# google/neural-light-transport

Hardware: NVIDIA B200
Metric: UV texels/sec fwd+bwd (higher is better)
Workload: dtype f32

## Files before the change

neural-light-transport_b200/csrc/nlt_tc.cu:

```cuda
#include <cuda.h>
#include "nlt_common.cuh"

namespace nlt {

constexpr int TC_MAX_STAGES = 8;
constexpr int TC_BM = 128;
constexpr int TC_EPI_PAD = 36;
constexpr int TC_EPI_BYTES = 4 * 32 * TC_EPI_PAD * 4;
constexpr int TC_THREADS = 320;
constexpr int TCF_THREADS = 448;
constexpr uint32_t TC_SPIN_LIMIT = 1u << 28;
unsigned long long g_tc_launches = 0;

int g_opt_tc_rawhi = -1;

struct TcParams {
  int N, Hl, Wl;
  int TW, TH;
  int tiles_x, tiles_y;
  int n_tiles_n;
  int total_tiles;
  int ntap_y, ntap_x;
  int nseg;
  int seg_chunks[NLT_MAX_SEG];
// ... 604 lines not shown
    const int lq = lane % QPR, lr = lane / QPR;

    struct Coord { int n, ty0, tx0, nt; };
    auto tile_coord = [&](int tile) {
      Coord c;
      const int mt = (int)fdiv((uint32_t)tile, p.div_ntn);
      c.nt = tile - mt * p.n_tiles_n;
      c.n = (int)fdiv((uint32_t)mt, p.div_tpi);
      const int r = mt - c.n * tiles_per_img;
      const int rq = (int)fdiv((uint32_t)r, p.div_tx);
      c.ty0 = rq * p.TH; c.tx0 = (r - rq * p.tiles_x) * p.TW;
      return c;
    };
    auto out_off = [&](const Coord& c, int row, int nb) -> size_t {
      const int rty = (int)fdiv((uint32_t)row, p.div_tw);
      const int ty = c.ty0 + rty, tx = c.tx0 + row - rty * p.TW;
      int cb = nb, oy, ox;
      if (p.d2s) {
        const int tap = (int)fdiv((uint32_t)nb, p.div_ct);
        cb = nb - tap * p.cout_true;
        const int dy = (int)fdiv((uint32_t)tap, p.div_s);
        oy = ty * p.d2s_s + dy; ox = tx * p.d2s_s + (tap - dy * p.d2s_s);
      } else {
        oy = p.o0y + p.osy * ty; ox = p.o0x + p.osx * tx;
      }
      return (((size_t)c.n * p.Hout + oy) * p.Wout + ox) * p.cout_true + cb;
    };
    float4 rm_old[NPASS], rm_y[NPASS];
    auto prefetch = [&](const Coord& c, int ch) {
#pragma unroll
      for (int i = 0; i < NPASS; ++i) {
        const size_t ob = out_off(c, quarter * 32 + i * RPI + lr, c.nt * BN + ch * 32 + lq * 4);
        rm_old[i] = (p.beta != 0.f) ? *reinterpret_cast<const float4*>(p.out + ob) : make_float4(0.f, 0.f, 0.f, 0.f);
        rm_y[i] = (p.mask_y != nullptr) ? ld4(p.mask_y + ob) : make_float4(1.f, 1.f, 1.f, 1.f);
      }
    };
    int it = 0;
    for (int tile = blockIdx.x; tile < p.total_tiles; tile += gridDim.x, ++it) {
      const int buf = it & 1;
      const uint32_t acc_phase = (uint32_t)(it >> 1) & 1;
      const Coord tc = tile_coord(tile);
      const uint32_t taddr = tmem_base + ((uint32_t)(quarter * 32) << 16) + (uint32_t)(buf * BN);
#pragma unroll 1
      for (int ch = 0; ch < NCH; ++ch) {
        if (rmw) prefetch(tc, ch);
        if (ch == 0) {
          mbar_wait(bar_accf(buf), acc_phase);
          tc_fence_after();
        }
        const int col0 = tc.nt * BN + ch * 32;
#pragma unroll
        for (int h = 0; h < CW / 16; ++h) {
          uint32_t v[16];
          tc_ld16(taddr + ch * 32 + h * 16, v);
#pragma unroll
          for (int q4 = 0; q4 < 4; ++q4) {
            int cb = col0 + h * 16 + q4 * 4;
            if (p.d2s) cb -= (int)fdiv((uint32_t)cb, p.div_ct) * p.cout_true;
            float o[4];
#pragma unroll
            for (int e = 0; e < 4; ++e) {
              float x = __uint_as_float(v[q4 * 4 + e]);
              if (p.bias != nullptr) x += __ldg(p.bias + cb + e);
              o[e] = act_fwd(x, p.act);
            }
            *reinterpret_cast<float4*>(stg + lane * TC_EPI_PAD + h * 16 + q4 * 4) = make_float4(o[0], o[1], o[2], o[3]);
          }
        }
        __syncwarp();
#pragma unroll
        for (int i = 0; i < NPASS; ++i) {
          const int row = i * RPI + lr;
          float4 o = *reinterpret_cast<const float4*>(stg + row * TC_EPI_PAD + lq * 4);
          if (rmw) {
            o.x += p.beta * rm_old[i].x; o.y += p.beta * rm_old[i].y; o.z += p.beta * rm_old[i].z; o.w += p.beta * rm_old[i].w;
            if (p.mask_y != nullptr) {
              o.x *= act_bwd_from_y(rm_y[i].x, p.mask_act); o.y *= act_bwd_from_y(rm_y[i].y, p.mask_act);
              o.z *= act_bwd_from_y(rm_y[i].z, p.mask_act); o.w *= act_bwd_from_y(rm_y[i].w, p.mask_act);
            }
          }
          const size_t ob = out_off(tc, quarter * 32 + row, col0 + lq * 4);
          *reinterpret_cast<float4*>(p.out + ob) = o;
        }
        __syncwarp();
      }
      tc_fence_before();
      mbar_arrive(bar_acce(buf));
    }
  }

  tc_fence_before();
  __syncthreads();
  if (warp == 1) {
    tc_fence_after();
    asm volatile("tcgen05.dealloc.cta_group::1.sync.aligned.b32 %0, %1;" ::"r"(tmem_base), "r"(TMEM_COLS) : "memory");
  }
}

typedef CUresult (*EncodeTiledFn)(CUtensorMap*, CUtensorMapDataType, cuuint32_t, void*, const cuuint64_t*,
                                  const cuuint64_t*, const cuuint32_t*, const cuuint32_t*, CUtensorMapInterleave,
                                  CUtensorMapSwizzle, CUtensorMapL2promotion, CUtensorMapFloatOOBfill);

static EncodeTiledFn get_encode() {
  static EncodeTiledFn fn = nullptr;
  static bool tried = false;
  if (!tried) {
    tried = true;
    void* sym = nullptr;
    cudaDriverEntryPointQueryResult qres;
    if (cudaGetDriverEntryPoint("cuTensorMapEncodeTiled", &sym, cudaEnableDefault, &qres) == cudaSuccess &&
        qres == cudaDriverEntryPointSuccess)
      fn = (EncodeTiledFn)sym;
  }
  return fn;
}

struct TcPlan {
  bool ok;
  bool ts;
  int bn;
  int kbw;
  TcParams p;
  int chunks_per_tap;
  int cout_pad;
  size_t pack_floats;
  size_t smem_bytes;
};

static int pick_bn(int cout) {
  if (cout % 128 == 0) return 128;
  if (cout % 64 == 0) return 64;
  if (cout % 32 == 0) return 32;
  if (cout % 16 == 0) return 16;
  return 0;
}

int g_opt_tcs = -1;
static int g_tcs_kmin = -1;
static bool tcs_enabled() {
  if (g_opt_tcs < 0) { const char* e = getenv("NLT_TCS"); g_opt_tcs = e ? (atoi(e) != 0) : NLT_TCS_DEFAULT; }
  if (g_tcs_kmin < 0) { const char* e = getenv("NLT_TCS_KMIN"); g_tcs_kmin = e ? atoi(e) : 64; }
  return g_opt_tcs == 1;
}

static TcPlan tc_plan(const GConvK& k) {
  TcPlan pl;
  memset(&pl, 0, sizeof(pl));
  pl.ok = false;
  const bool ts = tcs_enabled();
  pl.ts = ts;
  if (k.cout_true % 4 != 0) return pl;
  pl.bn = pick_bn(k.Cout);
  if (pl.bn == 0) return pl;
  int ctot = 0;
  pl.kbw = 32;
  for (int s = 0; s < k.nseg; ++s) {
    const Seg& sg = k.seg[s];
    if (sg.C % 16 != 0 || sg.sub != nullptr || sg.bcast || !aligned16(sg.ptr)) return pl;
    if (sg.C % 32 != 0) pl.kbw = 16;
    ctot += sg.C;
  }
  const int TC_KB = pl.kbw;
  if (!aligned16(k.w)) {  }
  if (ts) {
    if (k.ay.nu * k.ax.nu * ctot < g_tcs_kmin) return pl;
  } else {
    if (k.ay.nu * k.ax.nu * ctot < 64) return pl;
    if (pl.kbw == 16 && k.ay.nu * k.ax.nu * ctot < 128) return pl;
  }
  if (k.ay.nu < 1 || k.ax.nu < 1) return pl;
  TcParams& p = pl.p;
  p.N = k.N; p.Hl = k.ay.nt; p.Wl = k.ax.nt;
  if (p.Wl >= TC_BM) {
    if (p.Wl % TC_BM) return pl;
    p.TW = TC_BM; p.TH = 1;
  } else {
    if (TC_BM % p.Wl) return pl;
    p.TW = p.Wl; p.TH = TC_BM / p.Wl;
    if (p.Hl % p.TH) return pl;
  }
  p.tiles_x = p.Wl / p.TW; p.tiles_y = p.Hl / p.TH;
  const bool stride1 = (k.ay.it == 1 && k.ax.it == 1);
  const bool patch = (!k.d2s && k.ay.it > 1 && k.ay.it == k.ax.it && k.ay.iu == 1 && k.ax.iu == 1 && k.ay.i0 == 0 &&
                      k.ax.i0 == 0 && k.ay.nu == k.ay.it && k.ax.nu == k.ax.it && k.Hin == k.ay.nt * k.ay.it &&
                      k.Win == k.ax.nt * k.ax.it);
  if (!stride1 && !patch) return pl;
  p.mode_patch = patch ? 1 : 0;
  p.ux_step = k.ax.iu; p.x_off = k.ax.i0; p.uy_step = k.ay.iu; p.y_off = k.ay.i0;
  p.Hs = patch ? k.Hin / k.ay.it : 0;
  if (patch && (k.ay.it > 256 || p.TW > 256)) return pl;
  p.ntap_y = k.ay.nu; p.ntap_x = k.ax.nu;
  p.nseg = k.nseg;
  pl.chunks_per_tap = 0;
  for (int s = 0; s < k.nseg; ++s) { p.seg_chunks[s] = k.seg[s].C / TC_KB; pl.chunks_per_tap += p.seg_chunks[s]; }
  p.kb_total = p.ntap_y * p.ntap_x * pl.chunks_per_tap;
  p.Hout = k.Hout; p.Wout = k.Wout; p.cout_true = k.cout_true; p.Cout = k.Cout;
  p.o0y = k.ay.o0; p.osy = k.ay.os; p.o0x = k.ax.o0; p.osx = k.ax.os;
  p.d2s = k.d2s; p.d2s_s = k.d2s_s;
  static int split_waves = -1;
  if (split_waves < 0) { const char* e = getenv("NLT_TC_SPLIT_WAVES"); split_waves = (e && e[0] == '1') ? 1 : 0; }
  while (pl.bn > 32) {
    const long long tiles = (long long)p.N * p.tiles_x * p.tiles_y * (k.Cout / pl.bn);
    if (split_waves ? tiles >= 148 : 2 * tiles > 148) break;
    pl.bn /= 2;
  }
  p.n_tiles_n = k.Cout / pl.bn;
  p.div_ntn = make_fastdiv((uint32_t)p.n_tiles_n); p.div_tpi = make_fastdiv((uint32_t)(p.tiles_x * p.tiles_y));
  p.div_tx = make_fastdiv((uint32_t)p.tiles_x); p.div_tw = make_fastdiv((uint32_t)p.TW);
  p.div_ct = make_fastdiv((uint32_t)p.cout_true); p.div_s = make_fastdiv((uint32_t)(p.d2s ? p.d2s_s : 1));
  const long long tt = (long long)p.N * p.tiles_x * p.tiles_y * p.n_tiles_n;
  if (tt > (1ll << 30)) return pl;
  p.total_tiles = (int)tt;
  pl.cout_pad = k.Cout;
  pl.pack_floats = (size_t)p.kb_total * pl.cout_pad * TC_KB;
  {
    const size_t stage_bytes = (ts ? 1 : 2) * (size_t)TC_BM * TC_KB * 4 + 2 * (size_t)pl.bn * TC_KB * 4;
    int st = (int)((227 * 1024 - TC_EPI_BYTES - 2048) / stage_bytes);
    if (st > TC_MAX_STAGES) st = TC_MAX_STAGES;
    if (st < 2) return pl;
    p.stages = st;
    pl.smem_bytes = (size_t)st * stage_bytes + TC_EPI_BYTES + 1024;
  }
  if (get_encode() == nullptr) return pl;
  {
    static int ablate = -1;
    if (ablate < 0) {
      const char* e = getenv("NLT_TC_ABLATE");
      ablate = e ? atoi(e) : 0;
      if (ablate & 32) { const int one = 1; cudaMemcpyToSymbol(g_tc_poll, &one, sizeof(int)); }
    }
    p.ablate = ablate;
    if (g_opt_tc_rawhi < 0) { const char* e = getenv("NLT_TC_RAWHI"); g_opt_tc_rawhi = (e && e[0] == '0') ? 0 : 1; }
    p.rawhi = g_opt_tc_rawhi;
  }
  pl.ok = true;
  return pl;
}

static int encode_maps(const GConvK& k, const TcPlan& pl, const float* bhi, const float* blo, TcMaps* maps) {
  EncodeTiledFn enc = get_encode();
  const TcParams& p = pl.p;
  const int TC_KB = pl.kbw;
  const CUtensorMapSwizzle swz = pl.kbw == 32 ? CU_TENSOR_MAP_SWIZZLE_128B : CU_TENSOR_MAP_SWIZZLE_64B;
  for (int s = 0; s < k.nseg; ++s) {
    const Seg& sg = k.seg[s];
    const cuuint64_t C = sg.C, W = k.Win, H = k.Hin, N = k.N;
    CUresult r;
    if (p.mode_patch) {
      const cuuint64_t st = k.ay.it;
      cuuint64_t dims[5] = {C, st, W / st, st, N * (H / st)};
      cuuint64_t strides[4] = {C * 4, st * C * 4, W * C * 4, st * W * C * 4};
      cuuint32_t box[5] = {(cuuint32_t)TC_KB, 1, (cuuint32_t)p.TW, 1, (cuuint32_t)p.TH};
      cuuint32_t es[5] = {1, 1, 1, 1, 1};
      r = enc(&maps->a[s], CU_TENSOR_MAP_DATA_TYPE_FLOAT32, 5, (void*)sg.ptr, dims, strides, box, es,
              CU_TENSOR_MAP_INTERLEAVE_NONE, swz, CU_TENSOR_MAP_L2_PROMOTION_L2_128B,
              CU_TENSOR_MAP_FLOAT_OOB_FILL_NONE);
    } else {
      cuuint64_t dims[4] = {C, W, H, N};
      cuuint64_t strides[3] = {C * 4, W * C * 4, H * W * C * 4};
      cuuint32_t box[4] = {(cuuint32_t)TC_KB, (cuuint32_t)p.TW, (cuuint32_t)p.TH, 1};
      cuuint32_t es[4] = {1, 1, 1, 1};
      r = enc(&maps->a[s], CU_TENSOR_MAP_DATA_TYPE_FLOAT32, 4, (void*)sg.ptr, dims, strides, box, es,
              CU_TENSOR_MAP_INTERLEAVE_NONE, swz, CU_TENSOR_MAP_L2_PROMOTION_L2_128B,
              CU_TENSOR_MAP_FLOAT_OOB_FILL_NONE);
    }
    if (r != CUDA_SUCCESS) return set_err(NLT_ERR_CUDA, "cuTensorMapEncodeTiled(A seg %d) failed: %d", s, (int)r);
  }
  const float* planes[2] = {bhi, blo};
  CUtensorMap* bm[2] = {&maps->bhi, &maps->blo};
  for (int i = 0; i < 2; ++i) {
    cuuint64_t dims[3] = {(cuuint64_t)TC_KB, (cuuint64_t)pl.cout_pad, (cuuint64_t)p.kb_total};
    cuuint64_t strides[2] = {(cuuint64_t)TC_KB * 4, (cuuint64_t)TC_KB * 4 * pl.cout_pad};
    cuuint32_t box[3] = {(cuuint32_t)TC_KB, (cuuint32_t)pl.bn, 1};
    cuuint32_t es[3] = {1, 1, 1};
    CUresult r = enc(bm[i], CU_TENSOR_MAP_DATA_TYPE_FLOAT32, 3, (void*)planes[i], dims, strides, box, es,
                     CU_TENSOR_MAP_INTERLEAVE_NONE, swz, CU_TENSOR_MAP_L2_PROMOTION_L2_256B,
                     CU_TENSOR_MAP_FLOAT_OOB_FILL_NONE);
    if (r != CUDA_SUCCESS) return set_err(NLT_ERR_CUDA, "cuTensorMapEncodeTiled(B) failed: %d", (int)r);
  }
  return NLT_OK;
}

constexpr int WG_PT = 32;
constexpr int WG_MAX_PIECES = 36;
constexpr int WG_PLANE_A = TC_BM * 128;

struct WgPiece {
  int16_t is_g, seg, uy, ux;
  int16_t c0, w;
  int16_t row, pad;
  int32_t raw_off;
};

struct WgParams {
  int N, Hl, Wl, TW, TH, tiles_x, tiles_y, total_ptiles;
  int mode_patch, ux_step, x_off, uy_step, y_off, Hs;
  int g_patch, g_px, g_py, g_Hs;
  int g_ct, g_s;
  int ntap_x, nseg, ctot, Kd;
  int seg_C[NLT_MAX_SEG], seg_coff[NLT_MAX_SEG];
  int n_mtiles, n_ntiles;
  FastDiv div_tpi, div_tx;
  int raw_stages, raw_stage_bytes;
  int Cout, ld, KD_pad, bias_row;
  float* ws;
};

struct WgMaps {
  CUtensorMap a[NLT_MAX_SEG][4];
  CUtensorMap g;
};

__device__ __forceinline__ int wg_wclass(int w) { return w == 32 ? 3 : w == 16 ? 2 : w == 8 ? 1 : 0; }

__device__ __forceinline__ int wg_raw_chunk(int w, int p, int cq) {
  return w == 32 ? (cq ^ (p & 7)) : w == 16 ? (cq ^ ((p >> 1) & 3)) : w == 8 ? (cq ^ ((p >> 2) & 1)) : cq;
}

template <int BN>
__global__ void __launch_bounds__(TC_THREADS, 1)
tc_wgrad_kernel(const __grid_constant__ WgMaps maps, const WgParams p) {
  constexpr int PLANE_G = BN * 128;
  constexpr int PLANES_BYTES = 2 * WG_PLANE_A + 2 * PLANE_G;
  constexpr uint32_t TMEM_COLS = BN <= 32 ? 32 : BN <= 64 ? 64 : 128;
  constexpr uint32_t IDESC = (1u << 4) | (2u << 7) | (2u << 10) | ((uint32_t)(BN >> 3) << 17) | ((uint32_t)(TC_BM >> 4) << 24);
  constexpr int GQ = BN / 4;
  constexpr int GI = (GQ + 3) / 4;

  extern __shared__ uint8_t smem_raw[];
  uint8_t* smem = smem_raw + ((1024u - (smem_u32(smem_raw) & 1023u)) & 1023u);
  __shared__ __align__(8) uint64_t bars[2 * TC_MAX_STAGES + 5];
  __shared__ uint32_t tmem_base_smem;
  __shared__ WgPiece pieces[WG_MAX_PIECES];
  __shared__ uint16_t items[64];
  __shared__ int n_pieces_s, n_items_s, raw_bytes_s;
  __shared__ float bias_part[64];

  const int S = p.raw_stages;
  const int warp = threadIdx.x >> 5, lane = threadIdx.x & 31;
  const uint32_t bar0 = smem_u32(bars);
  auto bar_rfull = [&](int s) { return bar0 + 8u * s; };
  auto bar_rempty = [&](int s) { return bar0 + 8u * (TC_MAX_STAGES + s); };
  auto bar_tready = [&](int b) { return bar0 + 8u * (2 * TC_MAX_STAGES + b); };
  auto bar_tempty = [&](int b) { return bar0 + 8u * (2 * TC_MAX_STAGES + 2 + b); };
  const uint32_t bar_accf = bar0 + 8u * (2 * TC_MAX_STAGES + 4);
  uint8_t* planes = smem;
  uint8_t* raw = smem + 2 * PLANES_BYTES;
  const uint32_t planes_u32 = smem_u32(planes), raw_u32 = smem_u32(raw);

  const int mtile = blockIdx.y, ntile = blockIdx.z;
  const int k_lo = mtile * TC_BM, k_hi = min(p.Kd, k_lo + TC_BM);

  if (threadIdx.x == 0) {
    int np = 0, off = 0, k = k_lo;
    while (k < k_hi) {
      const int tap = k / p.ctot, c = k - tap * p.ctot;
      int s = 0;
      while (s < p.nseg - 1 && c >= p.seg_coff[s] + p.seg_C[s]) ++s;
      const int cin = c - p.seg_coff[s];
      int w = p.seg_C[s] - cin;
      if (w > 32) w = 32;
      if (w > k_hi - k) w = k_hi - k;
      w = w >= 32 ? 32 : w >= 16 ? 16 : w >= 8 ? 8 : 4;
      WgPiece& pc = pieces[np++];
      pc.is_g = 0; pc.seg = (int16_t)s; pc.uy = (int16_t)(tap / p.ntap_x); pc.ux = (int16_t)(tap % p.ntap_x);
      pc.c0 = (int16_t)cin; pc.w = (int16_t)w; pc.row = (int16_t)(k - k_lo); pc.pad = 0; pc.raw_off = off;
      off += (WG_PT * w * 4 + 1023) & ~1023;
      k += w;
    }
    const int gw = p.g_patch == 2 ? min(min(BN, 32), p.g_ct) : (BN < 32 ? BN : 32);
    for (int c = 0; c < BN; c += gw) {
      WgPiece& pc = pieces[np++];
      pc.is_g = 1; pc.seg = 0; pc.uy = 0; pc.ux = 0; pc.c0 = (int16_t)(ntile * BN + c); pc.w = (int16_t)gw;
      if (p.g_patch == 2) {
        const int ncol = ntile * BN + c, tap = ncol / p.g_ct;
        pc.c0 = (int16_t)(ncol - tap * p.g_ct);
        pc.uy = (int16_t)(tap / p.g_s); pc.ux = (int16_t)(tap % p.g_s);
      }
      pc.row = (int16_t)c; pc.pad = 0; pc.raw_off = off;
      off += (WG_PT * gw * 4 + 1023) & ~1023;
    }
    n_pieces_s = np;
    int bytes = 0, ni = 0;
    for (int i = 0; i < np; ++i) {
      bytes += WG_PT * pieces[i].w * 4;
      for (int cq = 0; cq < pieces[i].w / 4; ++cq) items[ni++] = (uint16_t)((i << 8) | cq);
    }
    n_items_s = ni;
    raw_bytes_s = bytes;
    for (int s = 0; s < S; ++s) { mbar_init(bar_rfull(s), 1); mbar_init(bar_rempty(s), 8); }
    for (int b = 0; b < 2; ++b) { mbar_init(bar_tready(b), 8); mbar_init(bar_tempty(b), 1); }
    mbar_init(bar_accf, 1);
    asm volatile("fence.mbarrier_init.release.cluster;" ::: "memory");
  }
  for (int i = threadIdx.x; i < 2 * PLANES_BYTES / 16; i += TC_THREADS)
    reinterpret_cast<float4*>(planes)[i] = make_float4(0.f, 0.f, 0.f, 0.f);
  if (warp == 1) {
    asm volatile("tcgen05.alloc.cta_group::1.sync.aligned.shared::cta.b32 [%0], %1;" ::"r"(smem_u32(&tmem_base_smem)),
                 "r"(TMEM_COLS) : "memory");
    asm volatile("tcgen05.relinquish_alloc_permit.cta_group::1.sync.aligned;" ::: "memory");
  }
  asm volatile("fence.proxy.async.shared::cta;" ::: "memory");
  tc_fence_before();
  __syncthreads();
  tc_fence_after();
  const uint32_t tmem_base = tmem_base_smem;
  const int n_pieces = n_pieces_s;
  const int tiles_per_img = p.tiles_x * p.tiles_y;
  int my_tiles = 0;
  for (int t = blockIdx.x; t < p.total_ptiles; t += gridDim.x) ++my_tiles;

  if (warp == 0) {
    if (lane == 0) {
      int stage = 0;
      uint32_t phase = 0;
      for (int t = blockIdx.x; t < p.total_ptiles; t += gridDim.x) {
        const int n = (int)fdiv((uint32_t)t, p.div_tpi);
        const int r = t - n * tiles_per_img;
        const int rq = (int)fdiv((uint32_t)r, p.div_tx);
        const int ty0 = rq * p.TH, tx0 = (r - rq * p.tiles_x) * p.TW;
        mbar_wait(bar_rempty(stage), phase ^ 1);
        mbar_expect_tx(bar_rfull(stage), (uint32_t)raw_bytes_s);
        const uint32_t base = raw_u32 + (uint32_t)stage * p.raw_stage_bytes;
        for (int i = 0; i < n_pieces; ++i) {
          const WgPiece pc = pieces[i];
          if (pc.is_g) {
            if (p.g_patch == 2)
              tma_load_5d(base + pc.raw_off, &maps.g, bar_rfull(stage), pc.c0, pc.ux, tx0, pc.uy, n * p.g_Hs + ty0);
            else if (p.g_patch)
              tma_load_5d(base + pc.raw_off, &maps.g, bar_rfull(stage), pc.c0, p.g_px, tx0, p.g_py, n * p.g_Hs + ty0);
            else
              tma_load_4d(base + pc.raw_off, &maps.g, bar_rfull(stage), pc.c0, tx0, ty0, n);
          } else {
            const CUtensorMap* m = &maps.a[pc.seg][wg_wclass(pc.w)];
            if (p.mode_patch)
              tma_load_5d(base + pc.raw_off, m, bar_rfull(stage), pc.c0, pc.ux, tx0, pc.uy, n * p.Hs + ty0);
            else
              tma_load_4d(base + pc.raw_off, m, bar_rfull(stage), pc.c0, tx0 + pc.ux * p.ux_step + p.x_off,
                          ty0 + pc.uy * p.uy_step + p.y_off, n);
          }
        }
        if (++stage == S) { stage = 0; phase ^= 1; }
      }
    }
  } else if (warp == 1) {
    if (lane == 0) {
      for (int i = 0; i < my_tiles; ++i) {
        const int b = i & 1;
        mbar_wait(bar_tready(b), (uint32_t)(i >> 1) & 1);
        tc_fence_after();
        const uint32_t ahi = planes_u32 + (uint32_t)b * PLANES_BYTES, alo = ahi + WG_PLANE_A;
        const uint32_t ghi = alo + WG_PLANE_A, glo = ghi + PLANE_G;
#pragma unroll
        for (int ks = 0; ks < WG_PT / 8; ++ks) {
          const uint64_t dah = umma_desc_kmajor<128>(ahi + ks * 32), dal = umma_desc_kmajor<128>(alo + ks * 32);
          const uint64_t dgh = umma_desc_kmajor<128>(ghi + ks * 32), dgl = umma_desc_kmajor<128>(glo + ks * 32);
          tc_mma_tf32(tmem_base, dal, dgh, IDESC, (i | ks) != 0);
          tc_mma_tf32(tmem_base, dah, dgl, IDESC, 1);
          tc_mma_tf32(tmem_base, dah, dgh, IDESC, 1);
        }
        tc_commit(bar_tempty(b));
        if (i == my_tiles - 1) tc_commit(bar_accf);
      }
    }
  } else {
    const int t = threadIdx.x - 64;
    const int px = t & 31, ql = t >> 5;
    const int n_items = n_items_s;
    constexpr int MAXI = 6;
    float gsum[MAXI][4];
#pragma unroll
    for (int i = 0; i < MAXI; ++i) { gsum[i][0] = gsum[i][1] = gsum[i][2] = gsum[i][3] = 0.f; }
    const int pxc = px >> 2, pxo = (px & 3) << 2;
    int stage = 0;
    uint32_t phase = 0;
    for (int it = 0; it < my_tiles; ++it) {
      const int b = it & 1;
      mbar_wait(bar_rfull(stage), phase);
      mbar_wait(bar_tempty(b), ((uint32_t)(it >> 1) & 1) ^ 1);
      const uint8_t* rbase = raw + (size_t)stage * p.raw_stage_bytes;
      uint8_t* pl = planes + (size_t)b * PLANES_BYTES;
#pragma unroll
      for (int i = 0; i < MAXI; ++i) {
        const int j = ql + 8 * i;
        if (j >= n_items) break;
        const int itm = items[j];
        const WgPiece pc = pieces[itm >> 8];
        const int cq = itm & 0xff;
        uint8_t* hi = pl + (pc.is_g ? 2 * WG_PLANE_A : 0);
        const int lo_off = pc.is_g ? PLANE_G : WG_PLANE_A;
        const float4 v = *reinterpret_cast<const float4*>(rbase + pc.raw_off + (size_t)px * pc.w * 4 +
                                                          wg_raw_chunk(pc.w, px, cq) * 16);
        const float vv[4] = {v.x, v.y, v.z, v.w};
        if (pc.is_g) { gsum[i][0] += v.x; gsum[i][1] += v.y; gsum[i][2] += v.z; gsum[i][3] += v.w; }
        const int row0 = pc.row + cq * 4;
        const int r7 = row0 & 7;
#pragma unroll
        for (int e = 0; e < 4; ++e) {
          const int o = (row0 + e) * 128 + (((pxc ^ (r7 + e)) << 4) | pxo);
          const float h = tf32_round(vv[e]);
          *reinterpret_cast<float*>(hi + o) = h;
          *reinterpret_cast<float*>(hi + lo_off + o) = tf32_round(vv[e] - h);
        }
      }
      asm volatile("fence.proxy.async.shared::cta;" ::: "memory");
      __syncwarp();
      if (lane == 0) {
        mbar_arrive(bar_tready(b));
        mbar_arrive(bar_rempty(stage));
      }
      if (++stage == S) { stage = 0; phase ^= 1; }
    }
#pragma unroll
    for (int i = 0; i < MAXI; ++i) {
      const int j = ql + 8 * i;
      const bool isg = j < n_items && pieces[items[j < n_items ? j : 0] >> 8].is_g;
#pragma unroll
      for (int e = 0; e < 4; ++e) {
        float v = gsum[i][e];
#pragma unroll
        for (int o = 16; o > 0; o >>= 1) v += __shfl_xor_sync(0xffffffffu, v, o);
        if (isg && px == 0) {
          const int itm = items[j];
          bias_part[pieces[itm >> 8].row + (itm & 0xff) * 4 + e] = v;
        }
      }
    }
  }
  __syncthreads();
  if (warp >= 6) {
    const int quarter = warp & 3;
    const int r = quarter * 32 + lane;
    const int k = k_lo + r;
    if (my_tiles > 0) {
      mbar_wait(bar_accf, 0);
      tc_fence_after();
    }
    float* dst = p.ws + ((size_t)blockIdx.x * p.KD_pad + (k < k_hi ? k : 0)) * p.ld + ntile * BN;
    const uint32_t taddr = tmem_base + ((uint32_t)(quarter * 32) << 16);
#pragma unroll 1
    for (int c0 = 0; c0 < BN; c0 += 16) {
      uint32_t v[16];
      if (my_tiles > 0) {
        tc_ld16(taddr + c0, v);
      } else {
#pragma unroll
        for (int e = 0; e < 16; ++e) v[e] = 0u;
      }
      if (k < k_hi) {
#pragma unroll
        for (int q4 = 0; q4 < 4; ++q4)
          *reinterpret_cast<float4*>(dst + c0 + q4 * 4) =
              make_float4(__uint_as_float(v[q4 * 4]), __uint_as_float(v[q4 * 4 + 1]), __uint_as_float(v[q4 * 4 + 2]),
                          __uint_as_float(v[q4 * 4 + 3]));
      }
    }
    if (mtile == 0 && r < BN)
      p.ws[((size_t)blockIdx.x * p.KD_pad + p.bias_row) * p.ld + ntile * BN + r] = my_tiles > 0 ? bias_part[r] : 0.f;
  }
  tc_fence_before();
  __syncthreads();
  if (warp == 1) {
    tc_fence_after();
    asm volatile("tcgen05.dealloc.cta_group::1.sync.aligned.b32 %0, %1;" ::"r"(tmem_base), "r"(TMEM_COLS) : "memory");
  }
}

struct WgPlan {
  bool ok;
  int bn;
  WgParams p;
  size_t smem_bytes;
  int nsplit;
};

static WgPlan wg_plan(const GConvK& k) {
  WgPlan pl;
  memset(&pl, 0, sizeof(pl));
  if (k.M == 0 || k.Cout % 16 != 0) return pl;
  if (k.d2s && (k.cout_true % 4 != 0 || (k.cout_true & (k.cout_true - 1)) != 0) && k.cout_true % 32 != 0) return pl;
  int ctot = 0;
  for (int s = 0; s < k.nseg; ++s) {
    const Seg& sg = k.seg[s];
    if (sg.C % 4 != 0 || sg.sub != nullptr || sg.bcast || !aligned16(sg.ptr)) return pl;
    ctot += sg.C;
  }
  if (k.ay.nu < 1 || k.ax.nu < 1) return pl;
  pl.bn = k.Cout % 64 == 0 ? 64 : k.Cout % 32 == 0 ? 32 : 16;
  WgParams& p = pl.p;
  p.N = k.N; p.Hl = k.ay.nt; p.Wl = k.ax.nt;
  if (p.Wl >= WG_PT) {
    if (p.Wl % WG_PT) return pl;
    p.TW = WG_PT; p.TH = 1;
  } else {
    if (WG_PT % p.Wl) return pl;
    p.TW = p.Wl; p.TH = WG_PT / p.Wl;
    if (p.Hl % p.TH) return pl;
  }
  p.tiles_x = p.Wl / p.TW; p.tiles_y = p.Hl / p.TH;
  p.div_tpi = make_fastdiv((uint32_t)(p.tiles_x * p.tiles_y)); p.div_tx = make_fastdiv((uint32_t)p.tiles_x);
  const long long tt = (long long)p.N * p.tiles_x * p.tiles_y;
  if (tt > (1ll << 30) || tt < 4) return pl;
  p.total_ptiles = (int)tt;
  const bool stride1 = (k.ay.it == 1 && k.ax.it == 1);
  const bool patch = (k.ay.it > 1 && k.ay.it == k.ax.it && k.ay.iu == 1 && k.ax.iu == 1 && k.ay.i0 == 0 && k.ax.i0 == 0 &&
                      k.ay.nu == k.ay.it && k.ax.nu == k.ax.it && k.Hin == k.ay.nt * k.ay.it && k.Win == k.ax.nt * k.ax.it);
  if (!stride1 && !patch) return pl;
  p.mode_patch = patch ? 1 : 0;
  p.ux_step = k.ax.iu; p.x_off = k.ax.i0; p.uy_step = k.ay.iu; p.y_off = k.ay.i0;
  p.Hs = patch ? k.Hin / k.ay.it : 0;
  if (k.ay.os != k.ax.os) return pl;
  if (k.d2s) {
    if (k.Hout != p.Hl * k.d2s_s || k.Wout != p.Wl * k.d2s_s) return pl;
    p.g_patch = 2; p.g_py = 0; p.g_px = 0; p.g_Hs = k.Hout / k.d2s_s; p.g_ct = k.cout_true; p.g_s = k.d2s_s;
  } else if (k.ay.os == 1) {
    if (k.ay.o0 != 0 || k.ax.o0 != 0 || k.Hout != p.Hl || k.Wout != p.Wl) return pl;
    p.g_patch = 0;
  } else {
    const int os = k.ay.os;
    if (k.Hout != p.Hl * os || k.Wout != p.Wl * os) return pl;
    p.g_patch = 1; p.g_py = k.ay.o0; p.g_px = k.ax.o0; p.g_Hs = k.Hout / os;
  }
  p.ntap_x = k.ax.nu; p.nseg = k.nseg; p.ctot = ctot;
  p.Kd = k.ay.nu * k.ax.nu * ctot;
  if (p.Kd < 128) return pl;
  int coff = 0;
  for (int s = 0; s < k.nseg; ++s) { p.seg_C[s] = k.seg[s].C; p.seg_coff[s] = coff; coff += k.seg[s].C; }
  p.n_mtiles = (p.Kd + TC_BM - 1) / TC_BM;
  p.n_ntiles = k.Cout / pl.bn;
  p.Cout = k.Cout; p.ld = k.Cout;
  p.bias_row = p.Kd; p.KD_pad = p.Kd + 4;
  p.raw_stage_bytes = 32 * 1024 + 8 * 1024;
  {
    int bytes = 0, kk = 0;
    const int k_hi = p.Kd < TC_BM ? p.Kd : TC_BM;
    int worst = 0;
    for (int mt = 0; mt < p.n_mtiles; ++mt) {
      bytes = 0; kk = mt * TC_BM;
      const int hi = (kk + TC_BM < p.Kd) ? kk + TC_BM : p.Kd;
      while (kk < hi) {
        const int tap = kk / ctot, c = kk - tap * ctot;
        int s = 0;
        while (s < k.nseg - 1 && c >= p.seg_coff[s] + p.seg_C[s]) ++s;
        int w = p.seg_C[s] - (c - p.seg_coff[s]);
        if (w > 32) w = 32;
        if (w > hi - kk) w = hi - kk;
        w = w >= 32 ? 32 : w >= 16 ? 16 : w >= 8 ? 8 : 4;
        bytes += (WG_PT * w * 4 + 1023) & ~1023;
        kk += w;
      }
      if (bytes > worst) worst = bytes;
    }
    (void)k_hi;
    int gw = pl.bn < 32 ? pl.bn : 32;
    if (k.d2s && k.cout_true < gw) gw = k.cout_true;
    worst += (pl.bn / gw) * ((WG_PT * gw * 4 + 1023) & ~1023);
    p.raw_stage_bytes = worst;
  }
  const size_t planes = 2 * (2 * (size_t)WG_PLANE_A + 2 * (size_t)pl.bn * 128);
  int st = (int)((227 * 1024 - 2048 - (long long)planes - 4096) / p.raw_stage_bytes);
  if (st > TC_MAX_STAGES) st = TC_MAX_STAGES;
  if (st < 2) return pl;
  p.raw_stages = st;
  pl.smem_bytes = planes + (size_t)st * p.raw_stage_bytes + 1024;
  long long want = 148 / ((long long)p.n_mtiles * p.n_ntiles);
  if (want < 1) want = 1;
  if (want > tt / 4) want = tt / 4;
  if (want < 1) want = 1;
  pl.nsplit = (int)want;
  if (get_encode() == nullptr) return pl;
  pl.ok = true;
  return pl;
}

bool tc_wgrad_applicable(const GConvK& k) { return wg_plan(k).ok; }

size_t tc_wgrad_ws_floats(const GConvK& k) {
  WgPlan pl = wg_plan(k);
  return pl.ok ? (size_t)pl.nsplit * pl.p.KD_pad * pl.p.ld : 0;
}

template <int BN>
static int wg_launch(const WgMaps& maps, const WgPlan& pl, cudaStream_t st) {
  static bool attr_set[64] = {false};
  int dev = 0;
  cudaGetDevice(&dev);
  if (dev < 0 || dev >= 64 || !attr_set[dev]) {
    cudaError_t e = cudaFuncSetAttribute(tc_wgrad_kernel<BN>, cudaFuncAttributeMaxDynamicSharedMemorySize, 227 * 1024 - 4096);
    if (e != cudaSuccess) return set_err(NLT_ERR_CUDA, "cudaFuncSetAttribute: %s", cudaGetErrorString(e));
    if (dev >= 0 && dev < 64) attr_set[dev] = true;
  }
  dim3 grid(pl.nsplit, pl.p.n_mtiles, pl.p.n_ntiles);
  tc_wgrad_kernel<BN><<<grid, TC_THREADS, pl.smem_bytes, st>>>(maps, pl.p);
  NLT_CUDA_LAUNCH_CHECK("tc_wgrad_kernel");
  __atomic_add_fetch(&g_tc_launches, 1ull, __ATOMIC_RELAXED);
  return NLT_OK;
}

static CUresult wg_encode(EncodeTiledFn enc, CUtensorMap* m, const float* ptr, int C, int W, int H, int N, int w, int TW,
                          int TH, int patch_s) {
  const CUtensorMapSwizzle swz = w == 32 ? CU_TENSOR_MAP_SWIZZLE_128B : w == 16 ? CU_TENSOR_MAP_SWIZZLE_64B
                                 : w == 8 ? CU_TENSOR_MAP_SWIZZLE_32B : CU_TENSOR_MAP_SWIZZLE_NONE;
  const cuuint64_t c = C, ww = W, h = H, n = N;
  if (patch_s > 1) {
    const cuuint64_t st_ = patch_s;
    cuuint64_t dims[5] = {c, st_, ww / st_, st_, n * (h / st_)};
    cuuint64_t strides[4] = {c * 4, st_ * c * 4, ww * c * 4, st_ * ww * c * 4};
    cuuint32_t box[5] = {(cuuint32_t)w, 1, (cuuint32_t)TW, 1, (cuuint32_t)TH};
    cuuint32_t es[5] = {1, 1, 1, 1, 1};
    return enc(m, CU_TENSOR_MAP_DATA_TYPE_FLOAT32, 5, (void*)ptr, dims, strides, box, es, CU_TENSOR_MAP_INTERLEAVE_NONE,
               swz, CU_TENSOR_MAP_L2_PROMOTION_L2_128B, CU_TENSOR_MAP_FLOAT_OOB_FILL_NONE);
  }
  cuuint64_t dims[4] = {c, ww, h, n};
  cuuint64_t strides[3] = {c * 4, ww * c * 4, h * ww * c * 4};
  cuuint32_t box[4] = {(cuuint32_t)w, (cuuint32_t)TW, (cuuint32_t)TH, 1};
  cuuint32_t es[4] = {1, 1, 1, 1};
  return enc(m, CU_TENSOR_MAP_DATA_TYPE_FLOAT32, 4, (void*)ptr, dims, strides, box, es, CU_TENSOR_MAP_INTERLEAVE_NONE, swz,
             CU_TENSOR_MAP_L2_PROMOTION_L2_128B, CU_TENSOR_MAP_FLOAT_OOB_FILL_NONE);
}

int launch_tc_wgrad(const GConvK& k, const float* G, float* ws, WgradK* w, size_t* KD_pad, cudaStream_t st) {
  WgPlan pl = wg_plan(k);
  if (!pl.ok) return set_err(NLT_ERR_INVALID, "tensor-core wgrad not applicable");
  NLT_CHECK_ARG(aligned16(G), "dz must be 16-byte aligned");
  EncodeTiledFn enc = get_encode();
  WgMaps maps;
  memset(&maps, 0, sizeof(maps));
  const WgParams& p = pl.p;
  static const int widths[4] = {4, 8, 16, 32};
  for (int s = 0; s < k.nseg; ++s)
    for (int wi = 0; wi < 4; ++wi) {
      if (widths[wi] > k.seg[s].C) continue;
      CUresult r = wg_encode(enc, &maps.a[s][wi], k.seg[s].ptr, k.seg[s].C, k.Win, k.Hin, k.N, widths[wi], p.TW, p.TH,
                             p.mode_patch ? k.ay.it : 1);
      if (r != CUDA_SUCCESS) return set_err(NLT_ERR_CUDA, "cuTensorMapEncodeTiled(wgrad A %d/%d) failed: %d", s, widths[wi], (int)r);
    }
  {
    int gw = pl.bn < 32 ? pl.bn : 32;
    if (k.d2s && k.cout_true < gw) gw = k.cout_true;
    CUresult r = k.d2s ? wg_encode(enc, &maps.g, G, k.cout_true, k.Wout, k.Hout, k.N, gw, p.TW, p.TH, k.d2s_s)
                       : wg_encode(enc, &maps.g, G, k.Cout, k.Wout, k.Hout, k.N, gw, p.TW, p.TH, p.g_patch ? k.ay.os : 1);
    if (r != CUDA_SUCCESS) return set_err(NLT_ERR_CUDA, "cuTensorMapEncodeTiled(wgrad G) failed: %d", (int)r);
  }
  pl.p.ws = ws;
  w->g = k;
  w->GS = p.ctot / 4;
  w->KG = k.ay.nu * k.ax.nu * w->GS + 1;
  w->ld = p.ld; w->nsplit = pl.nsplit; w->pix_per_split = 0;
  *KD_pad = (size_t)p.KD_pad;
  switch (pl.bn) {
    case 64: return wg_launch<64>(maps, pl, st);
    case 32: return wg_launch<32>(maps, pl, st);
    default: return wg_launch<16>(maps, pl, st);
  }
}

bool tc_applicable(const GConvK& k) { return tc_plan(k).ok; }

size_t tc_workspace_bytes(const GConvK& k) {
  TcPlan pl = tc_plan(k);
  return pl.ok ? 2 * pl.pack_floats * sizeof(float) + 256 : 0;
}

template <int BN, int KBW>
static int tc_launch_bn(const TcMaps& maps, const TcPlan& pl, cudaStream_t st) {
  static bool attr_set[2][64] = {{false}};
  int dev = 0;
  cudaGetDevice(&dev);
  if (dev < 0 || dev >= 64 || !attr_set[pl.ts ? 1 : 0][dev]) {
    cudaError_t e = pl.ts ? cudaFuncSetAttribute(tcs_gconv_kernel<BN, KBW>, cudaFuncAttributeMaxDynamicSharedMemorySize,
                                                 227 * 1024 - 1024)
                          : cudaFuncSetAttribute(tc_gconv_kernel<BN, KBW>, cudaFuncAttributeMaxDynamicSharedMemorySize,
                                                 227 * 1024 - 1024);
    if (e != cudaSuccess) return set_err(NLT_ERR_CUDA, "cudaFuncSetAttribute: %s", cudaGetErrorString(e));
    if (dev >= 0 && dev < 64) attr_set[pl.ts ? 1 : 0][dev] = true;
  }
  const int grid = pl.p.total_tiles < 148 ? pl.p.total_tiles : 148;
  if (pl.ts) tcs_gconv_kernel<BN, KBW><<<grid, TCF_THREADS, pl.smem_bytes, st>>>(maps, pl.p);
  else tc_gconv_kernel<BN, KBW><<<grid, TCF_THREADS, pl.smem_bytes, st>>>(maps, pl.p);
  NLT_CUDA_LAUNCH_CHECK("tc_gconv_kernel");
  __atomic_add_fetch(&g_tc_launches, 1ull, __ATOMIC_RELAXED);
  return NLT_OK;
}

int tc_pack(const GConvK& k, void* workspace, size_t workspace_bytes, cudaStream_t st) {
  TcPlan pl = tc_plan(k);
  if (!pl.ok) return set_err(NLT_ERR_INVALID, "tensor-core path not applicable");
  const size_t need = 2 * pl.pack_floats * sizeof(float) + 256;
  NLT_CHECK_ARG(workspace != nullptr && workspace_bytes >= need, "tc workspace too small: need %zu", need);
  float* bhi = reinterpret_cast<float*>((reinterpret_cast<uintptr_t>(workspace) + 255) & ~(uintptr_t)255);
  float* blo = bhi + pl.pack_floats;
  const size_t total = pl.pack_floats;
  int blocks = (int)((total + 255) / 256);
  if (blocks > 148 * 8) blocks = 148 * 8;
  tc_pack_weights_kernel<<<blocks, 256, 0, st>>>(k, pl.kbw, pl.p.kb_total, pl.chunks_per_tap, pl.cout_pad, bhi, blo);
  NLT_CUDA_LAUNCH_CHECK("tc_pack_weights_kernel");
  return NLT_OK;
}

int launch_tc(const GConvK& k, const float* bias, int act, float beta, const float* mask_y, int mask_act, float* out,
              void* workspace, size_t workspace_bytes, cudaStream_t st, bool prepacked) {
  TcPlan pl = tc_plan(k);
  if (!pl.ok) return set_err(NLT_ERR_INVALID, "tensor-core path not applicable");
  const size_t need = 2 * pl.pack_floats * sizeof(float) + 256;
  NLT_CHECK_ARG(workspace != nullptr && workspace_bytes >= need, "tc workspace too small: need %zu", need);
  float* bhi = reinterpret_cast<float*>((reinterpret_cast<uintptr_t>(workspace) + 255) & ~(uintptr_t)255);
  float* blo = bhi + pl.pack_floats;
  if (!prepacked) {
    const int rc0 = tc_pack(k, workspace, workspace_bytes, st);
    if (rc0 != NLT_OK) return rc0;
  }
  TcMaps maps;
  int rc = encode_maps(k, pl, bhi, blo, &maps);
  if (rc != NLT_OK) return rc;
  pl.p.act = act; pl.p.mask_act = mask_act; pl.p.beta = beta; pl.p.bias = bias; pl.p.mask_y = mask_y; pl.p.out = out;
  if (pl.kbw == 32) {
    switch (pl.bn) {
      case 128: return tc_launch_bn<128, 32>(maps, pl, st);
      case 64: return tc_launch_bn<64, 32>(maps, pl, st);
      case 32: return tc_launch_bn<32, 32>(maps, pl, st);
      default: return tc_launch_bn<16, 32>(maps, pl, st);
    }
  }
  switch (pl.bn) {
    case 128: return tc_launch_bn<128, 16>(maps, pl, st);
    case 64: return tc_launch_bn<64, 16>(maps, pl, st);
    case 32: return tc_launch_bn<32, 16>(maps, pl, st);
    default: return tc_launch_bn<16, 16>(maps, pl, st);
  }
}

}
```

Measured before the change: 642.5 million.

## Add MN-major tcgen05 weight-gradient kernel using 3xTF32 with swizzled TMA tiles

```diff
diff --git a/neural-light-transport_b200/csrc/nlt_tc.cu b/neural-light-transport_b200/csrc/nlt_tc.cu
--- a/neural-light-transport_b200/csrc/nlt_tc.cu
+++ b/neural-light-transport_b200/csrc/nlt_tc.cu
@@ -930,6 +930,7 @@
   int n_mtiles, n_ntiles;
   FastDiv div_tpi, div_tx;
   int raw_stages, raw_stage_bytes;
+  int nacc;
   int Cout, ld, KD_pad, bias_row;
   float* ws;
 };
@@ -1194,8 +1195,235 @@
   }
 }
 
+constexpr int WM_PT = 16;
+constexpr int WM_BOX = WM_PT * 128;
+constexpr int WM_MAX_ABOX = 8;
+
+__device__ __forceinline__ int wm_logical_chunk(int pc, int r) { return pc ^ ((r & 3) << 1); }
+
+__device__ __forceinline__ uint64_t umma_desc_mn32(uint32_t smem_addr, uint32_t lbo) {
+  uint64_t d = 0;
+  d |= (uint64_t)((smem_addr & 0x3FFFF) >> 4);
+  d |= (uint64_t)(lbo >> 4) << 16;
+  d |= (uint64_t)(512 >> 4) << 32;
+  d |= (uint64_t)1 << 46;
+  d |= (uint64_t)1 << 61;
+  return d;
+}
+
+template <int BN>
+__global__ void __launch_bounds__(TC_THREADS, 1)
+tc_wgrad_mn_kernel(const __grid_constant__ WgMaps maps, const WgParams p) {
+  constexpr int NG = BN / 32;
+  constexpr uint32_t IDESC = (1u << 4) | (2u << 7) | (2u << 10) | (1u << 15) | (1u << 16) | ((uint32_t)(BN >> 3) << 17) |
+                             ((uint32_t)(TC_BM >> 4) << 24);
+  extern __shared__ uint8_t smem_raw[];
+  uint8_t* smem = smem_raw + ((1024u - (smem_u32(smem_raw) & 1023u)) & 1023u);
+  __shared__ __align__(8) uint64_t bars[3 * TC_MAX_STAGES + 1];
+  __shared__ uint32_t tmem_base_smem;
+  __shared__ int4 abox[WM_MAX_ABOX];
+
+  const int S = p.raw_stages, nacc = p.nacc;
+  const int GA = 4 * nacc;
+  const int stage_bytes = 2 * (GA + NG) * WM_BOX;
+  const int lo_off = (GA + NG) * WM_BOX;
+  const uint32_t tmem_cols = nacc * BN <= 32 ? 32 : nacc * BN <= 64 ? 64 : nacc * BN <= 128 ? 128 : nacc * BN <= 256 ? 256 : 512;
+  const int warp = threadIdx.x >> 5, lane = threadIdx.x & 31;
+  const uint32_t bar0 = smem_u32(bars);
+  auto bar_full = [&](int s) { return bar0 + 8u * s; };
+  auto bar_ready = [&](int s) { return bar0 + 8u * (TC_MAX_STAGES + s); };
+  auto bar_empty = [&](int s) { return bar0 + 8u * (2 * TC_MAX_STAGES + s); };
+  const uint32_t bar_accf = bar0 + 8u * (3 * TC_MAX_STAGES);
+  const uint32_t smem_base = smem_u32(smem);
+
+  const int mgroup = blockIdx.y, ntile = blockIdx.z;
+  const int k_lo = mgroup * GA * 32;
+  const int na = min(GA, (p.Kd - k_lo) / 32);
+
+  if (threadIdx.x == 0) {
+    for (int j = 0; j < na; ++j) {
+      const int kr = k_lo + 32 * j, tap = kr / p.ctot, c = kr - tap * p.ctot;
+      int s = 0;
+      while (s < p.nseg - 1 && c >= p.seg_coff[s] + p.seg_C[s]) ++s;
+      abox[j] = make_int4(s, c - p.seg_coff[s], tap / p.ntap_x, tap % p.ntap_x);
+    }
+    for (int s = 0; s < S; ++s) {
+      mbar_init(bar_full(s), 1);
+      mbar_init(bar_ready(s), 8);
+      mbar_init(bar_empty(s), 1);
+    }
+    mbar_init(bar_accf, 1);
+    asm volatile("fence.mbarrier_init.release.cluster;" ::: "memory");
+  }
+  if (na < GA) {
+    for (int i = threadIdx.x; i < S * stage_bytes / 16; i += TC_THREADS)
+      reinterpret_cast<float4*>(smem)[i] = make_float4(0.f, 0.f, 0.f, 0.f);
+    asm volatile("fence.proxy.async.shared::cta;" ::: "memory");
+  }
+  if (warp == 1) {
+    asm volatile("tcgen05.alloc.cta_group::1.sync.aligned.shared::cta.b32 [%0], %1;" ::"r"(smem_u32(&tmem_base_smem)),
+                 "r"(tmem_cols) : "memory");
+    asm volatile("tcgen05.relinquish_alloc_permit.cta_group::1.sync.aligned;" ::: "memory");
+  }
+  tc_fence_before();
+  __syncthreads();
+  tc_fence_after();
+  const uint32_t tmem_base = tmem_base_smem;
+  const int tiles_per_img = p.tiles_x * p.tiles_y;
+  const int my_tiles = (p.total_ptiles - (int)blockIdx.x + (int)gridDim.x - 1) / (int)gridDim.x;
+
+  if (warp == 0) {
+    if (lane == 0) {
+      int stage = 0;
+      uint32_t phase = 0;
+      for (int t = blockIdx.x; t < p.total_ptiles; t += gridDim.x) {
+        const int n = (int)fdiv((uint32_t)t, p.div_tpi);
+        const int r = t - n * tiles_per_img;
+        const int rq = (int)fdiv((uint32_t)r, p.div_tx);
+        const int ty0 = rq * p.TH, tx0 = (r - rq * p.tiles_x) * p.TW;
+        mbar_wait(bar_empty(stage), phase ^ 1);
+        mbar_expect_tx(bar_full(stage), (uint32_t)((na + NG) * WM_BOX));
+        const uint32_t base = smem_base + (uint32_t)(stage * stage_bytes);
+        for (int j = 0; j < na; ++j) {
+          const int4 b = abox[j];
+          if (p.mode_patch)
+            tma_load_5d(base + j * WM_BOX, &maps.a[b.x][0], bar_full(stage), b.y, b.w, tx0, b.z, n * p.Hs + ty0);
+          else
+            tma_load_4d(base + j * WM_BOX, &maps.a[b.x][0], bar_full(stage), b.y, tx0 + b.w * p.ux_step + p.x_off,
+                        ty0 + b.z * p.uy_step + p.y_off, n);
+        }
+#pragma unroll
+        for (int j = 0; j < NG; ++j) {
+          const uint32_t dst = base + (GA + j) * WM_BOX;
+          const int ncol = ntile * BN + 32 * j;
+          if (p.g_patch == 2) {
+            const int tap = ncol / p.g_ct;
+            tma_load_5d(dst, &maps.g, bar_full(stage), ncol - tap * p.g_ct, tap % p.g_s, tx0, tap / p.g_s, n * p.g_Hs + ty0);
+          } else if (p.g_patch) {
+            tma_load_5d(dst, &maps.g, bar_full(stage), ncol, p.g_px, tx0, p.g_py, n * p.g_Hs + ty0);
+          } else {
+            tma_load_4d(dst, &maps.g, bar_full(stage), ncol, tx0, ty0, n);
+          }
+        }
+        if (++stage == S) { stage = 0; phase ^= 1; }
+      }
+    }
+  } else if (warp == 1) {
+    if (lane == 0) {
+      int stage = 0;
+      uint32_t phase = 0;
+      const int nacc_live = (na + 3) / 4;
+      for (int i = 0; i < my_tiles; ++i) {
+        mbar_wait(bar_ready(stage), phase);
+        tc_fence_after();
+        const uint32_t base = smem_base + (uint32_t)(stage * stage_bytes);
+#pragma unroll
+        for (int ks = 0; ks < WM_PT / 8; ++ks) {
+          const uint32_t ko = ks * 8 * 128;
+          const uint64_t gh = umma_desc_mn32(base + GA * WM_BOX + ko, WM_BOX);
+          const uint64_t gl = umma_desc_mn32(base + lo_off + GA * WM_BOX + ko, WM_BOX);
+          for (int a = 0; a < nacc_live; ++a) {
+            const uint64_t ah = umma_desc_mn32(base + a * 4 * WM_BOX + ko, WM_BOX);
+            const uint64_t al = umma_desc_mn32(base + lo_off + a * 4 * WM_BOX + ko, WM_BOX);
+            const uint32_t d = tmem_base + (uint32_t)(a * BN);
+            tc_mma_tf32(d, al, gh, IDESC, (i | ks) != 0);
+            tc_mma_tf32(d, ah, gl, IDESC, 1);
+            tc_mma_tf32(d, ah, gh, IDESC, 1);
+          }
+        }
+        tc_commit(bar_empty(stage));
+        if (i == my_tiles - 1) tc_commit(bar_accf);
+        if (++stage == S) { stage = 0; phase ^= 1; }
+      }
+    }
+  } else {
+    const int t = threadIdx.x - 64;
+    const int nq = (GA + NG) * (WM_BOX / 16);
+    const int row = (t & 127) >> 3, pc = t & 7;
+    float4 gsum[(NG + 1) / 2];
+#pragma unroll
+    for (int j = 0; j < (NG + 1) / 2; ++j) gsum[j] = make_float4(0.f, 0.f, 0.f, 0.f);
+    int stage = 0;
+    uint32_t phase = 0;
+    for (int it = 0; it < my_tiles; ++it) {
+      mbar_wait(bar_full(stage), phase);
+      float4* raw = reinterpret_cast<float4*>(smem + (size_t)stage * stage_bytes);
+      float4* lo = reinterpret_cast<float4*>(smem + (size_t)stage * stage_bytes + lo_off);
+      for (int q = t; q < na * (WM_BOX / 16); q += 256) {
+        const float4 v = raw[q];
+        float4 l;
+        l.x = tf32_round(v.x - __uint_as_float(__float_as_uint(v.x) & 0xFFFFE000u));
+        l.y = tf32_round(v.y - __uint_as_float(__float_as_uint(v.y) & 0xFFFFE000u));
+        l.z = tf32_round(v.z - __uint_as_float(__float_as_uint(v.z) & 0xFFFFE000u));
+        l.w = tf32_round(v.w - __uint_as_float(__float_as_uint(v.w) & 0xFFFFE000u));
+        lo[q] = l;
+      }
+#pragma unroll
+      for (int j = 0; j < (NG + 1) / 2; ++j) {
+        const int q = GA * (WM_BOX / 16) + t + j * 256;
+        if (q < nq) {
+          const float4 v = raw[q];
+          float4 l;
+          l.x = tf32_round(v.x - __uint_as_float(__float_as_uint(v.x) & 0xFFFFE000u));
+          l.y = tf32_round(v.y - __uint_as_float(__float_as_uint(v.y) & 0xFFFFE000u));
+          l.z = tf32_round(v.z - __uint_as_float(__float_as_uint(v.z) & 0xFFFFE000u));
+          l.w = tf32_round(v.w - __uint_as_float(__float_as_uint(v.w) & 0xFFFFE000u));
+          lo[q] = l;
+          gsum[j].x += v.x; gsum[j].y += v.y; gsum[j].z += v.z; gsum[j].w += v.w;
+        }
+      }
+      asm volatile("fence.proxy.async.shared::cta;" ::: "memory");
+      __syncwarp();
+      if (lane == 0) mbar_arrive(bar_ready(stage));
+      if (++stage == S) { stage = 0; phase ^= 1; }
+    }
+    mbar_wait(bar_accf, 0);
+    float* stg = reinterpret_cast<float*>(smem);
+#pragma unroll
+    for (int j = 0; j < (NG + 1) / 2; ++j) {
+      const int gb = (t >> 7) + 2 * j;
+      if (gb < NG) {
+        float* d = stg + row * BN + gb * 32 + wm_logical_chunk(pc, row) * 4;
+        d[0] = gsum[j].x; d[1] = gsum[j].y; d[2] = gsum[j].z; d[3] = gsum[j].w;
+      }
+    }
+    asm volatile("bar.sync 1, 256;" ::: "memory");
+    if (mgroup == 0 && t < BN) {
+      float s = 0.f;
+#pragma unroll
+      for (int r = 0; r < WM_PT; ++r) s += stg[r * BN + t];
+      p.ws[((size_t)blockIdx.x * p.KD_pad + p.bias_row) * p.ld + ntile * BN + t] = s;
+    }
+    tc_fence_after();
+    const int quarter = warp & 3, half = (warp - 2) >> 2;
+    const uint32_t lane_base = tmem_base + ((uint32_t)(quarter * 32) << 16);
+    const int cols = nacc * BN;
+#pragma unroll 1
+    for (int c0 = half * 16; c0 < cols; c0 += 32) {
+      const int a = c0 / BN, cn = c0 - a * BN;
+      const int k = k_lo + a * TC_BM + quarter * 32 + lane;
+      uint32_t v[16];
+      tc_ld16(lane_base + c0, v);
+      if (k < p.Kd) {
+        float* dst = p.ws + ((size_t)blockIdx.x * p.KD_pad + k) * p.ld + ntile * BN + cn;
+#pragma unroll
+        for (int q4 = 0; q4 < 4; ++q4)
+          *reinterpret_cast<float4*>(dst + q4 * 4) = make_float4(__uint_as_float(v[q4 * 4]), __uint_as_float(v[q4 * 4 + 1]),
+                                                                 __uint_as_float(v[q4 * 4 + 2]), __uint_as_float(v[q4 * 4 + 3]));
+      }
+    }
+  }
+  tc_fence_before();
+  __syncthreads();
+  if (warp == 1) {
+    tc_fence_after();
+    asm volatile("tcgen05.dealloc.cta_group::1.sync.aligned.b32 %0, %1;" ::"r"(tmem_base), "r"(tmem_cols) : "memory");
+  }
+}
+
 struct WgPlan {
   bool ok;
+  bool mn;
   int bn;
   WgParams p;
   size_t smem_bytes;
@@ -1298,6 +1526,33 @@
   pl.nsplit = (int)want;
   if (get_encode() == nullptr) return pl;
   pl.ok = true;
+
+  bool mn = (k.d2s ? k.cout_true : k.Cout) % 32 == 0;
+  for (int s = 0; s < k.nseg; ++s) mn = mn && k.seg[s].C % 32 == 0;
+  if (!mn) return pl;
+  pl.mn = true;
+  pl.bn = k.Cout % 256 == 0 ? 256 : k.Cout % 128 == 0 ? 128 : k.Cout % 64 == 0 ? 64 : 32;
+  if (p.Wl >= WM_PT) { p.TW = WM_PT; p.TH = 1; }
+  else { p.TW = p.Wl; p.TH = WM_PT / p.Wl; }
+  p.tiles_x = p.Wl / p.TW; p.tiles_y = p.Hl / p.TH;
+  p.div_tpi = make_fastdiv((uint32_t)(p.tiles_x * p.tiles_y)); p.div_tx = make_fastdiv((uint32_t)p.tiles_x);
+  const long long ptiles = (long long)p.N * p.tiles_x * p.tiles_y;
+  p.total_ptiles = (int)ptiles;
+  p.n_ntiles = k.Cout / pl.bn;
+  const int mt128 = (p.Kd + TC_BM - 1) / TC_BM;
+  p.nacc = (mt128 >= 2 && (long long)mt128 * p.n_ntiles >= 16) ? 2 : 1;
+  p.n_mtiles = (mt128 + p.nacc - 1) / p.nacc;
+  const int stage_bytes = 2 * (4 * p.nacc + pl.bn / 32) * WM_BOX;
+  st = (227 * 1024 - 2048) / stage_bytes;
+  if (st > TC_MAX_STAGES) st = TC_MAX_STAGES;
+  if (st < 3) { pl.ok = false; return pl; }
+  p.raw_stages = st; p.raw_stage_bytes = stage_bytes;
+  pl.smem_bytes = (size_t)st * stage_bytes + 1024;
+  want = 148 / ((long long)p.n_mtiles * p.n_ntiles);
+  if (want > (4ll << 20) / ((long long)p.Kd * k.Cout)) want = (4ll << 20) / ((long long)p.Kd * k.Cout);
+  if (want > ptiles / 8) want = ptiles / 8;
+  if (want < 1) want = 1;
+  pl.nsplit = (int)want;
   return pl;
 }
 
@@ -1325,10 +1580,28 @@
   return NLT_OK;
 }
 
+template <int BN>
+static int wm_launch(const WgMaps& maps, const WgPlan& pl, cudaStream_t st) {
+  static bool attr_set[64] = {false};
+  int dev = 0;
+  cudaGetDevice(&dev);
+  if (dev < 0 || dev >= 64 || !attr_set[dev]) {
+    cudaError_t e = cudaFuncSetAttribute(tc_wgrad_mn_kernel<BN>, cudaFuncAttributeMaxDynamicSharedMemorySize, 227 * 1024 - 1024);
+    if (e != cudaSuccess) return set_err(NLT_ERR_CUDA, "cudaFuncSetAttribute: %s", cudaGetErrorString(e));
+    if (dev >= 0 && dev < 64) attr_set[dev] = true;
+  }
+  dim3 grid(pl.nsplit, pl.p.n_mtiles, pl.p.n_ntiles);
+  tc_wgrad_mn_kernel<BN><<<grid, TC_THREADS, pl.smem_bytes, st>>>(maps, pl.p);
+  NLT_CUDA_LAUNCH_CHECK("tc_wgrad_mn_kernel");
+  __atomic_add_fetch(&g_tc_launches, 1ull, __ATOMIC_RELAXED);
+  return NLT_OK;
+}
+
 static CUresult wg_encode(EncodeTiledFn enc, CUtensorMap* m, const float* ptr, int C, int W, int H, int N, int w, int TW,
-                          int TH, int patch_s) {
-  const CUtensorMapSwizzle swz = w == 32 ? CU_TENSOR_MAP_SWIZZLE_128B : w == 16 ? CU_TENSOR_MAP_SWIZZLE_64B
-                                 : w == 8 ? CU_TENSOR_MAP_SWIZZLE_32B : CU_TENSOR_MAP_SWIZZLE_NONE;
+                          int TH, int patch_s, bool mn) {
+  const CUtensorMapSwizzle swz = mn ? CU_TENSOR_MAP_SWIZZLE_128B_ATOM_32B : w == 32 ? CU_TENSOR_MAP_SWIZZLE_128B
+                                 : w == 16 ? CU_TENSOR_MAP_SWIZZLE_64B : w == 8 ? CU_TENSOR_MAP_SWIZZLE_32B
+                                 : CU_TENSOR_MAP_SWIZZLE_NONE;
   const cuuint64_t c = C, ww = W, h = H, n = N;
   if (patch_s > 1) {
     const cuuint64_t st_ = patch_s;
@@ -1357,17 +1630,18 @@
   const WgParams& p = pl.p;
   static const int widths[4] = {4, 8, 16, 32};
   for (int s = 0; s < k.nseg; ++s)
-    for (int wi = 0; wi < 4; ++wi) {
-      if (widths[wi] > k.seg[s].C) continue;
-      CUresult r = wg_encode(enc, &maps.a[s][wi], k.seg[s].ptr, k.seg[s].C, k.Win, k.Hin, k.N, widths[wi], p.TW, p.TH,
-                             p.mode_patch ? k.ay.it : 1);
-      if (r != CUDA_SUCCESS) return set_err(NLT_ERR_CUDA, "cuTensorMapEncodeTiled(wgrad A %d/%d) failed: %d", s, widths[wi], (int)r);
+    for (int wi = 0; wi < (pl.mn ? 1 : 4); ++wi) {
+      const int wd = pl.mn ? 32 : widths[wi];
+      if (wd > k.seg[s].C) continue;
+      CUresult r = wg_encode(enc, &maps.a[s][wi], k.seg[s].ptr, k.seg[s].C, k.Win, k.Hin, k.N, wd, p.TW, p.TH,
+                             p.mode_patch ? k.ay.it : 1, pl.mn);
+      if (r != CUDA_SUCCESS) return set_err(NLT_ERR_CUDA, "cuTensorMapEncodeTiled(wgrad A %d/%d) failed: %d", s, wd, (int)r);
     }
   {
     int gw = pl.bn < 32 ? pl.bn : 32;
     if (k.d2s && k.cout_true < gw) gw = k.cout_true;
-    CUresult r = k.d2s ? wg_encode(enc, &maps.g, G, k.cout_true, k.Wout, k.Hout, k.N, gw, p.TW, p.TH, k.d2s_s)
-                       : wg_encode(enc, &maps.g, G, k.Cout, k.Wout, k.Hout, k.N, gw, p.TW, p.TH, p.g_patch ? k.ay.os : 1);
+    CUresult r = k.d2s ? wg_encode(enc, &maps.g, G, k.cout_true, k.Wout, k.Hout, k.N, gw, p.TW, p.TH, k.d2s_s, pl.mn)
+                       : wg_encode(enc, &maps.g, G, k.Cout, k.Wout, k.Hout, k.N, gw, p.TW, p.TH, p.g_patch ? k.ay.os : 1, pl.mn);
     if (r != CUDA_SUCCESS) return set_err(NLT_ERR_CUDA, "cuTensorMapEncodeTiled(wgrad G) failed: %d", (int)r);
   }
   pl.p.ws = ws;
@@ -1376,6 +1650,14 @@
   w->KG = k.ay.nu * k.ax.nu * w->GS + 1;
   w->ld = p.ld; w->nsplit = pl.nsplit; w->pix_per_split = 0;
   *KD_pad = (size_t)p.KD_pad;
+  if (pl.mn) {
+    switch (pl.bn) {
+      case 256: return wm_launch<256>(maps, pl, st);
+      case 128: return wm_launch<128>(maps, pl, st);
+      case 64: return wm_launch<64>(maps, pl, st);
+      default: return wm_launch<32>(maps, pl, st);
+    }
+  }
   switch (pl.bn) {
     case 64: return wg_launch<64>(maps, pl, st);
     case 32: return wg_launch<32>(maps, pl, st);
```

New measurement: 657.9 million (median of 6 runs). +2.4%, better.
